# bistromath/gr-ais

Measured on AMD Instinct MI355X. Metric: complex MS/s through corr_est->msk_timing chain; corr_est %HBM roofline, higher is better.
Workload: dtype f32

## Files before the change

### __graft_entry__.py

```python
import os
import subprocess
import sys

ROOT = os.path.dirname(os.path.abspath(__file__))
for _p in (ROOT, os.path.join(ROOT, "gr-ais_amd"), os.path.join(ROOT, "tests")):
    if _p not in sys.path:
        sys.path.insert(0, _p)


def build():
    env = dict(os.environ)
    subprocess.check_call(["make", "-C", os.path.join(ROOT, "gr-ais_amd")], env=env)
    subprocess.check_call(["make", "-C", os.path.join(ROOT, "oracle")], env=env)
    for model in ("emul", "emul_hdlc", "emul_nmea", "emul_nmea_std", "emul_nmea_parse", "emul_msg", "emul_msg_enc", "emul_track", "emul_dedup", "emul_xlate", "emul_xlate_fmt",
                  "emul_mlse"):
        subprocess.check_call(["make", "-C", os.path.join(ROOT, "tests", model)], env=env)
    ub = os.path.join(ROOT, "tools", "ubench")
    src, exe = os.path.join(ub, "hbm_ceiling.hip"), os.path.join(ub, "hbm_ceiling")
    if not os.path.exists(exe) or os.path.getmtime(exe) < os.path.getmtime(src):
        subprocess.check_call([os.environ.get("HIPCC", "/opt/rocm/bin/hipcc"), "--offload-arch=gfx950", "-O3", "-o", exe, src], env=env)
    import ais_amd
    from ais_amd import _lib

    assert _lib.lib().aisx_version() >= 300


def smoke():
    import numpy as np
    import torch

# ... 36 lines not shown
```

### gr-ais_amd/ais_amd/_lib.py

```python
import ctypes as C
import os

_PKG = os.path.dirname(os.path.abspath(__file__))
LIB_VARIANT = os.environ.get("AISX_LIB_VARIANT", "")
LIB_PATH = os.path.join(os.path.dirname(_PKG), "lib", "libaisx_exp.so" if LIB_VARIANT == "exp" else "libaisx.so")

AISX_OK = 0
AISX_ERR_INVALID = -1
AISX_ERR_OUT_OF_RANGE = -2
AISX_ERR_HIP = -3
AISX_ERR_NO_DEVICE = -4
AISX_ERR_OVERFLOW = -5
AISX_ERR_RUNTIME = -6

AISX_FMT_CF32, AISX_FMT_CS16, AISX_FMT_CS8, AISX_FMT_CU8 = 0, 1, 2, 3
AISX_RX_ST_HDLC_OVERFLOW, AISX_RX_ST_NMEA_OVERFLOW, AISX_RX_ST_BAD_COUNT = 0x100, 0x200, 0x400
AISX_MSG_NA, AISX_MSG_STR = -(1 << 31), 48
AISX_HDLC_MAX_RULES = 16
AISX_HDLC_EV_SINGLE, AISX_HDLC_EV_PAIR, AISX_HDLC_EV_SKIP = 1, 2, 4
AISX_MLSE_ST_BAD_COUNT = 1
MLSE_BLOCK, MLSE_OVERLAP = 64, 16
AISX_MSG_FL_COMPLETE, AISX_MSG_FL_NO_LAYOUT, AISX_MSG_FL_BAD_RECORD = 1, 2, 4
AISX_MSG_ENC_NO_MMSI, AISX_MSG_ENC_NO_LAYOUT, AISX_MSG_ENC_RANGE, AISX_MSG_ENC_BAD_CHAR, AISX_MSG_ENC_BAD_ROW = 1, 2, 4, 8, 16
AISX_MSG_ENC_PITCH = 56
# ... 95 lines not shown
    sig("aisx_msk_process_stream", i32, [vp, vp, lng, i32, vp, vp, i32, vp, vp, vp, vp, lng, vp, vp])
    sig("aisx_msk_process_stream_after", i32, [vp, vp, lng, i32, vp, vp, i32, vp, vp, vp, vp, lng, vp, vp, vp])
    sig("aisx_msk_last_status", i32, [vp, pi32, vp])
    sig("aisx_msk_restart_stats", i32, [vp, vp, vp])
    sig("aisx_msk_set_profiling", i32, [vp, i32])
    sig("aisx_msk_kernel_ms_history", i32, [vp, C.POINTER(C.c_float), i32, pi32])
    sig("aisx_msk_set_max_noutput_items", i32, [vp, i32])
    sig("aisx_msk_set_time_parallel", i32, [vp, i32, i32, i32])
    sig("aisx_msk_get_max_noutput_items", i32, [vp])
    sig("aisx_msk_set_tail_stream", i32, [vp, vp, i32])
    sig("aisx_msk_wait_tail", i32, [vp, vp])
    sig("aisx_msk_set_fused_tail", i32, [vp, i32])
    sig("aisx_msk_get_fused_tail", i32, [vp])
    sig("aisx_msk_set_pair_core", i32, [vp, i32])
    sig("aisx_msk_get_pair_core", i32, [vp])
    sig("aisx_msk_last_tail_fused", i32, [vp])
    sig("aisx_msk_wait_prepass", i32, [vp, vp])
    sig("aisx_msk_set_head_start", i32, [vp, i32])
    sig("aisx_msk_geometry", i32, [vp, pi32, pi32])
    sig("aisx_msk_general_work_host", i32, [vp, i32, i32, vp, vp, vp, vp, vp, vp, i32, u64, i32, pi32, pi32])
    sig("aisx_freqsync_create", i32, [pvp, f64, f64, i32, i32, i32])
    sig("aisx_freqest_create", i32, [pvp, f32, i32, i32, i32])
    sig("aisx_freqest_create_n", i32, [pvp, f32, i32, i32, i32, i32])
    sig("aisx_freqsync_is_estimator_only", i32, [vp])
    sig("aisx_freqsync_geometry", i32, [vp, pi32, pi32, pi32])
    sig("aisx_freqsync_drop_ahead", i32, [vp, vp])
    sig("aisx_freqsync_destroy", i32, [vp])
    sig("aisx_freqsync_reset", i32, [vp])
    sig("aisx_freqsync_process", i32, [vp, vp, lng, i32, vp, lng, vp, lng, pi32, vp])
    sig("aisx_freqest_work", i32, [vp, vp, lng, vp, lng, i32, vp])
# ... 182 lines not shown
```

### gr-ais_amd/ais_amd/blocks.py

```python
import ctypes as C
import math

import numpy as np
import torch

from . import _lib
from ._lib import check

TAG_DTYPE = np.dtype([("offset", "<u8"), ("value", "<f8"), ("key", "<i4"), ("chan", "<i4")])


def _stream_ptr(stream=None):
    s = stream if stream is not None else torch.cuda.current_stream()
    return C.c_void_p(s.cuda_stream)


def _dev_c64(x, nchan):
    if not isinstance(x, torch.Tensor):
        x = torch.as_tensor(np.ascontiguousarray(x, dtype=np.complex64))
    if x.dtype != torch.complex64:
        raise TypeError("expected complex64 (gr_complex) items, got %s" % x.dtype)
    if not x.is_cuda:
        x = x.cuda()
    x = x.reshape(nchan, -1)
# ... 214 lines not shown

    def wait_tail(self, stream=None):
        check(_lib.lib().aisx_msk_wait_tail(self._h, _stream_ptr(stream)), "wait_tail")

    def set_fused_tail(self, on):
        check(_lib.lib().aisx_msk_set_fused_tail(self._h, 1 if on else 0), "set_fused_tail")

    def get_fused_tail(self):
        return bool(_lib.lib().aisx_msk_get_fused_tail(self._h))

    def set_pair_core(self, mode):
        check(_lib.lib().aisx_msk_set_pair_core(self._h, int(mode)), "set_pair_core")

    def get_pair_core(self):
        return int(_lib.lib().aisx_msk_get_pair_core(self._h))

    def last_tail_fused(self):
        return _lib.lib().aisx_msk_last_tail_fused(self._h) == 1

    def wait_prepass(self, stream=None):
        check(_lib.lib().aisx_msk_wait_prepass(self._h, _stream_ptr(stream)), "wait_prepass")

    def last_status(self, stream=None):
        st = C.c_int(0)
        check(_lib.lib().aisx_msk_last_status(self._h, C.byref(st), _stream_ptr(stream)), "last_status")
        return st.value

    def set_time_parallel(self, restart_points=64, join_kernel=-1, max_unit_items=0):
        check(_lib.lib().aisx_msk_set_time_parallel(self._h, int(restart_points), int(join_kernel), int(max_unit_items)),
              "set_time_parallel")
# ... 668 lines not shown
```

### gr-ais_amd/csrc/aisx_devctx.h

```cpp
#pragma once
#include <hip/hip_runtime.h>
#include "aisx_common.h"

namespace aisx {

struct DevCtx {
    static constexpr bool wave_lds_coherent = true;
    char* lds_;
    __device__ __forceinline__ int tid() const { return threadIdx.x; }
    __device__ __forceinline__ int nthreads() const { return blockDim.x; }
    __device__ __forceinline__ int bx() const { return blockIdx.x; }
    __device__ __forceinline__ int by() const { return blockIdx.y; }
    __device__ __forceinline__ char* lds() const { return lds_; }
    __device__ __forceinline__ void sync() const { __syncthreads(); }
    __device__ __forceinline__ void wave_sync() const { __builtin_amdgcn_wave_barrier(); }
    __device__ __forceinline__ void wave_lds_sync() const
    {
        asm volatile("" ::: "memory");
        __builtin_amdgcn_wave_barrier();
    }
    __device__ __forceinline__ void retire() const {}
    __device__ __forceinline__ unsigned long long ballot(bool p) const { return __builtin_amdgcn_ballot_w64(p); }
    __device__ __forceinline__ bool inv_ballot(unsigned long long m) const { return __builtin_amdgcn_inverse_ballot_w64(m); }
    typedef float v2f __attribute__((ext_vector_type(2)));
// ... 74 lines not shown
            const auto ra = __builtin_amdgcn_permlane32_swap(a, a, false, false);
            const auto rb = __builtin_amdgcn_permlane32_swap(b, b, false, false);
            lo = mk(__uint_as_float(ra[0]), __uint_as_float(rb[0]));
            hi = mk(__uint_as_float(ra[1]), __uint_as_float(rb[1]));
        }
    }
    static constexpr bool has_pair_core = true;
    struct PairK {
        unsigned long long roleM;
        unsigned rbase;
        float gain_omega, d_sps, limit, gain;
        unsigned rstep;
        unsigned ring;
        unsigned pmask, pbase;
        float rnd;
    };
    __device__ __forceinline__ void pair_core(const PairK& k, float& mu, float& omega, int& sb, unsigned& so, unsigned& waddr, v2f& acc,
                                              v2f& sE, v2f& s1, float& nlO) const
    {
        float t1, t3, t4;
        int t2;
        asm volatile(
            "v_add_f32 %[t3], %[mu], %[om]\n\t"
            "v_cvt_i32_f32 %[t2], %[t3]\n\t"
            "v_fract_f32 %[t1], %[t3]\n\t"
            "v_mad_u32_u24 %[t4], %[t2], %[rstep], %[sb]\n\t"
            "v_cndmask_b32_e64 %[t3], %[mu], %[t1], %[roleM]\n\t"
            "v_and_b32 %[t4], 0x3fc0, %[t4]\n\t"
            "v_fmamk_f32 %[t3], %[t3], 0x43000000, %[rnd]\n\t"
            "v_add_u32 %[t4], %[ring], %[t4]\n\t"
// ... 54 lines not shown
            "v_subrev_f32 v1, %[lim], v1\n\t"
            "v_sub_f32_e64 v0, |v0|, |v1|\n\t"
            "v_mul_f32 v0, 0.5, v0\n\t"
            "v_add_f32 %[om], %[dsps], v0\n\t"
            "v_add_f32 v2, v2, %[om]\n\t"
            "v_cvt_i32_f32 v3, v2\n\t"
            "v_fract_f32 %[mu], v2\n\t"
            "v_lshl_add_u32 %[sb], v3, 6, %[sb]"
            : [mu] "+v"(mu), [om] "+v"(omega), [sb] "+v"(sb), [so] "+v"(so), [waddr] "+v"(waddr), [acc] "+v"(acc), "={v[16:17]}"(sE),
              "+{v[24:25]}"(s1), [nlO] "=&v"(nlO), [t1] "=&v"(t1), [t2] "=&v"(t2), [t3] "=&v"(t3), [t4] "=&v"(t4)
            : [roleM] "s"(k.roleM), [rbase] "s"(k.rbase), [go] "s"(k.gain_omega), [dsps] "s"(k.d_sps), [lim] "s"(k.limit), [gain] "s"(k.gain),
              [rstep] "v"(k.rstep), [ring] "v"(k.ring), [pmask] "v"(k.pmask), [pbase] "v"(k.pbase), [rnd] "v"(k.rnd)
            : "memory", "v0", "v1", "v2", "v3", "v4", "v5", "v6", "v7", "v8", "v9", "v10", "v11", "v12", "v13", "v14", "v15", "v18", "v19",
              "v20", "v21", "v22", "v23");
    }
    __device__ __forceinline__ void xpose8_lane_hi(cf (&x)[8]) const
    {
        unsigned u[16];
#pragma unroll
        for (int k = 0; k < 8; k++) {
            u[2 * k] = __float_as_uint(x[k].re);
            u[2 * k + 1] = __float_as_uint(x[k].im);
        }
#pragma unroll
        for (int r = 0; r < 4; r++)
#pragma unroll
            for (int d = 0; d < 2; d++) {
                const auto q = __builtin_amdgcn_permlane32_swap(u[2 * r + d], u[2 * (r + 4) + d], false, false);
                u[2 * r + d] = q[0];
                u[2 * (r + 4) + d] = q[1];
// ... 201 lines not shown
```

### gr-ais_amd/csrc/aisx_msk.hip

```cpp
#include <math.h>
#include <stdlib.h>

#include <algorithm>
#include <vector>

#include "aisx_devctx.h"
#include "aisx_msk_impl.h"
#include "aisx_plan.h"
#include "aisx_tables.h"

using namespace aisx;

template <bool AUX, bool OSPS2, int LPW>
__global__ __launch_bounds__(64 * msk_waves(LPW)) void k_msk(MskParams p)
{
    extern __shared__ __attribute__((aligned(16))) char smem[];
    DevCtx cx{ smem };
#ifndef MSK_PRIO
#define MSK_PRIO 3
#endif
    __builtin_amdgcn_s_setprio(MSK_PRIO);
    msk_body<DevCtx, AUX, OSPS2, LPW>(cx, p);
}

template <int LPW>
__global__ __launch_bounds__(64 * msk_waves(LPW)) void k_msk_ff(MskParams p)
{
    extern __shared__ __attribute__((aligned(16))) char smem[];
    DevCtx cx{ smem };
    __builtin_amdgcn_s_setprio(MSK_PRIO);
    msk_body<DevCtx, false, false, LPW, true>(cx, p);
}

__global__ __launch_bounds__(64 * msk_waves(8)) void k_msk_core(MskParams p)
{
    extern __shared__ __attribute__((aligned(16))) char smem[];
    DevCtx cx{ smem };
    __builtin_amdgcn_s_setprio(MSK_PRIO);
    msk_body<DevCtx, false, false, 8, false, true>(cx, p);
}

__global__ __launch_bounds__(BT_T) void k_bittail(BitTailParams p)
{
    __shared__ __attribute__((aligned(16))) char smem[260 * 4];
    DevCtx cx{ smem };
    bittail_body(cx, p);
}

__global__ __launch_bounds__(64) void k_msk_headstart(unsigned ticks)
// ... 23 lines not shown
    const int v = li * 4 + (((p.err || p.mu_out) ? 2 : 0) | (p.osps == 2 ? 1 : 0));
    static const int pad = [] {
        const char* e = exp_env("AISX_MSK_LDS_PAD");
        return e ? atoi(e) * 1024 : 0;
    }();
    const int lds = std::min(msk_lds_bytes(p.lpw) + pad, 160 * 1024);
    kfn fn = fns[v];
    if (p.ff) {
        static const kfn ffs[5] = { k_msk_ff<16>, k_msk_ff<32>, k_msk_ff<64>, k_msk_ff<8>, k_msk_ff<4> };
        if (p.err || p.mu_out || p.osps == 2) {
            set_err("msk_launch: the join build has no err / mu ports and osps == 1");
            return AISX_ERR_INVALID;
        }
        fn = ffs[li];
    } else if (p.pair_core && v == 3 * 4) {
        fn = k_msk_core;
    }
    int rc = ensure_dyn_lds((const void*)fn, lds, "msk_timing_recovery_cc");
    if (rc != AISX_OK)
        return rc;
    hipLaunchKernelGGL(fn, dim3(nwg), dim3(64 * msk_waves(p.lpw)), lds, st, p);
    AISX_HIPCHK(hipGetLastError());
    return AISX_OK;
}

static int msk_check_geometry(float d_sps, float gain, float limit)
{
    const float wmin = d_sps - fabsf(limit), wmax = d_sps + fabsf(limit);
    if (!(wmin >= 0.5f) || msk_forecast(d_sps, 1) + 1 > aisx_msk::carry_cap || !(2.f * wmax + 3.f * fabsf(gain) <= 32.f)) {
        set_err("msk_timing_recovery: sps/2 = %g with limit %g and gain %g is outside what the gfx950 kernel is sized for "
                "(sps/2 - |limit| >= 0.5, forecast(1) < %d items, 2 (sps/2 + |limit|) + 3 |gain| <= 32)",
// ... 182 lines not shown
void aisx::msk_fill_common(aisx_msk* h, MskParams& p)
{
    msk_fill_state(h, p);
    p.osps = h->osps;
    p.ct = h->d_ct;
    p.ct_n = h->d_ct_n;
    p.ct_cap = h->ct_cap();
    p.lds_tab_off = msk_lds_taboff(h->lpw);
    p.lpw = h->lpw;
    p.lds_wave_stride = msk_lds_wave(h->lpw);
    p.tq_stride = h->lpw;
    p.tq_private = 0;
    p.lds_ring_off = msk_lds_ringoff(h->lpw);
    p.inline_tags = h->inline_tags;
    p.pair_core = h->pair_core;
    p.stream_mode = 1;
    p.gr_ninput = 0;
    p.gr_noutput = 0;
    p.ff = 0;
    p.nrst = nullptr;
    p.rst = nullptr;
    p.res = nullptr;
    p.pieces = nullptr;
    p.npieces = nullptr;
    p.ct_nc = nullptr;
}

static int msk_ct_reserve(aisx_msk* h, int need, hipStream_t st)
{
    if (h->d_ct && need <= h->ct_cap())
// ... 234 lines not shown
        return AISX_ERR_INVALID;
    h->fused_tail = on != 0;
    return AISX_OK;
}
extern "C" int aisx_msk_get_fused_tail(const aisx_msk* h) { return h ? (h->fused_tail ? 1 : 0) : AISX_ERR_INVALID; }
extern "C" int aisx_msk_last_tail_fused(const aisx_msk* h) { return h ? (h->last_fused ? 1 : 0) : AISX_ERR_INVALID; }

extern "C" int aisx_msk_set_pair_core(aisx_msk* h, int mode)
{
    if (!h || (mode != 0 && mode != 1))
        return AISX_ERR_INVALID;
    h->pair_core = mode;
    return AISX_OK;
}
extern "C" int aisx_msk_get_pair_core(const aisx_msk* h) { return h ? h->pair_core : AISX_ERR_INVALID; }

extern "C" int aisx_msk_wait_prepass(aisx_msk* h, void* stream)
{
    if (!h)
        return AISX_ERR_INVALID;
    if (!h->ev_prep)
        return h->ev_prep.ensure(hipEventDisableTiming);
    if (h->ev_prep_set) {
        AISX_HIPCHK(hipStreamWaitEvent((hipStream_t)stream, h->ev_prep, 0));
        if (h->head_start_ticks > 0) {
            hipLaunchKernelGGL(k_msk_headstart, dim3(1), dim3(64), 0, (hipStream_t)stream, h->head_start_ticks);
            AISX_HIPCHK(hipGetLastError());
        }
    }
    return AISX_OK;
// ... 165 lines not shown
```

### gr-ais_amd/csrc/aisx_msk_impl.h

```cpp
#pragma once
#include <memory>
#include <vector>

#include "aisx_host.h"
#include "k_msk.h"

#pragma GCC visibility push(hidden)
namespace aisx {
struct MskTp;
struct MskTpDelete {
    void operator()(MskTp* t) const;
};
}

struct aisx_msk {
    int nchan = 0, max_items = 0, out_cap = 0, osps = 1;
    aisx::EventRing prof;
    int lpw = 64;
    int inline_tags = 1;
    float d_sps = 0, gain = 0, gain_omega = 0, limit = 0;
    static constexpr int carry_cap = aisx::MSK_CARRY_MAX, ctag_cap = 64;
    aisx::DevBuf<float> d_mu, d_omega;
    aisx::DevBuf<int> d_div;
    aisx::DevBuf<aisx::cf> d_dly1, d_dly2, d_diff1;
    aisx::DevBuf<aisx::cf> d_tprev[2];
    aisx::DevBuf<unsigned char> d_tbit[2];
    int tcur = 0;
    aisx::DevBuf<aisx::cf> d_symscratch[2];
    int callpar = 0;
    bool tail_on = false;
    hipStream_t tail_stream = nullptr;
    aisx::Event ev_msk, ev_tail[2];
    unsigned head_start_ticks = 0;
    aisx::Event ev_prep;
    bool ev_prep_set = false;
    bool ev_tail_set[2] = { false, false };
    bool fused_tail = true, last_fused = false;
    int pair_core = 1;
    hipStream_t last_st = nullptr;
    bool tail_pend[2] = { false, false };
    aisx::DevBuf<int> d_produced2;
    aisx::DevBuf<unsigned long long> d_nread;
    aisx::DevBuf<aisx::cf> d_carry[2];
    aisx::DevBuf<int> d_carry_len[2];
    aisx::DevBuf<aisx::tag_rec> d_ctag[2];
    aisx::DevBuf<int> d_ctag_n[2];
    aisx::DevBuf<aisx::msk_ctag> d_ct;
    aisx::DevBuf<int> d_ct_n;
    int ct_cap() const { return (int)(d_ct.cap() / (size_t)nchan); }
    int cur = 0;
    aisx::DevBuf<int> d_produced, d_consumed, d_status;
    aisx::DevBuf<float> d_mmse, d_atan;
    int max_noutput = 0;
// ... 77 lines not shown
```

### gr-ais_amd/csrc/aisx_stages.hip

```cpp
#include <math.h>
#include <stdlib.h>
#include <string.h>

#include <vector>

#include "aisx_devctx.h"
#include "aisx_host.h"
#include "aisx_tables.h"
#include "k_agc.h"
#include "k_agcw.h"
#include "k_freqsync.h"

using namespace aisx;

__global__ __launch_bounds__(FS_T) void k_fs_est(FsEstParams p)
{
    extern __shared__ __attribute__((aligned(16))) char smem[];
    DevCtx cx{ smem };
    fs_est_body(cx, p);
}
__global__ __launch_bounds__(FSM_T) void k_fs_mix(FsMixParams p)
{
    extern __shared__ __attribute__((aligned(16))) char smem[];
    DevCtx cx{ smem };
// ... 273 lines not shown
extern "C" int aisx_freqsync_process(aisx_freqsync* h, const aisx_cf32* d_in, long in_stride, int n, aisx_cf32* d_out,
                                     long out_stride, float* d_fhat, long fhat_stride, int* n_out, void* stream)
{
    if (fs_whole(h, "aisx_freqsync_process") != AISX_OK)
        return AISX_ERR_INVALID;
    if (!h || !d_in || !d_out || !n_out || n < 1 || n > h->max_items || in_stride < n) {
        set_err("aisx_freqsync_process: bad argument");
        return AISX_ERR_INVALID;
    }
    hipStream_t st = (hipStream_t)stream;
    const int nvec = (h->npend + n) / h->fftlen;
    if (out_stride < (long)nvec * h->fftlen || (d_fhat && fhat_stride < nvec)) {
        set_err("aisx_freqsync_process: output stride too small for %d vectors", nvec);
        return AISX_ERR_INVALID;
    }
    h->ahead_cnt = 0;
    if (h->walk_pending)
        AISX_HIPCHK(hipStreamWaitEvent(st, h->ev_walk, 0));
    if (h->proc_pending)
        AISX_HIPCHK(hipStreamWaitEvent(st, h->ev_proc, 0));
    if (nvec > 0) {
        FsEstParams e;
        e.in = (const cf*)d_in;
        e.in_stride = in_stride;
        e.pend = h->d_pend[h->cur];
        e.npend = h->npend;
        e.wtab = h->d_wtab;
        e.maxpos = h->d_maxpos;
        e.maxpos_stride = h->max_vec;
        e.nvec = nvec;
// ... 10 lines not shown
    m.npend = h->npend;
    m.n = n;
    m.out = (cf*)d_out;
    m.out_stride = out_stride;
    m.maxpos = h->d_maxpos;
    m.maxpos_stride = h->max_vec;
    m.fhat = d_fhat;
    m.fhat_stride = fhat_stride;
    m.phase = h->d_phase;
    m.nvec = nvec;
    m.binsize = h->binsize;
    m.sensitivity = h->sensitivity;
    m.sintab = h->d_sintab;
    hipLaunchKernelGGL(k_fs_mix, dim3((h->nchan + FSM_CPW - 1) / FSM_CPW), dim3(FSM_T), FSM_LDS_BYTES, st, m);
    AISX_HIPCHK(hipGetLastError());
    if (h->ev_proc) {
        AISX_HIPCHK(hipEventRecord(h->ev_proc, st));
        AISX_HIPCHK(hipEventRecord(h->ev_walk, st));
        h->proc_pending = h->walk_pending = true;
        AISX_HIPCHK(hipEventRecord(h->slot[0].ev_read, st));
        h->slot[0].read_pending = true;
    }
    h->npend = h->npend + n - nvec * h->fftlen;
    h->cur ^= 1;
    *n_out = nvec * h->fftlen;
    return AISX_OK;
}

extern "C" int aisx_freqest_work(aisx_freqsync* h, const aisx_cf32* d_vecs, long vec_stride, float* d_out,
                                 long out_stride, int nvec, void* stream)
{
    if (!h || !d_vecs || !d_out || nvec < 0 || vec_stride < (long)nvec * h->fftlen || out_stride < nvec)
        return AISX_ERR_INVALID;
    if (nvec == 0)
        return AISX_OK;
    FsFreqestParams p;
    p.vecs = (const cf*)d_vecs;
// ... 571 lines not shown
```

### gr-ais_amd/csrc/k_msk.h

```cpp
#pragma once
#include "aisx_common.h"

namespace aisx {

enum {
    MSK_ST_INTERP_RANGE = 1,
    MSK_ST_CARRY_OVERFLOW = 2,
    MSK_ST_TAGCARRY_OVERFLOW = 4,
    MSK_ST_OUT_FULL = 8,
    MSK_ST_TAGS_TRUNCATED = 16
};
constexpr int MSK_CTN_TRUNC = 0x40000000;
constexpr int MSK_CTN_WILD = 0x20000000;
constexpr int MSK_TAG_TRIPS = 6;

constexpr int MSK_T = 64;
constexpr int MSK_RING = 256;
constexpr int MSK_SLOTS = MSK_RING + 8;
constexpr int MSK_CHUNK = 64;
constexpr int MSK_OFF = 192;
constexpr int MSK_CARRY_MAX = 128;
constexpr int MSK_PAIRS_MAX = 16;
#ifndef MSK_TRIP
#define MSK_TRIP 8
// ... 126 lines not shown
    int stream_mode; int gr_ninput; int gr_noutput;
    const msk_ctag* ct; const int* ct_n; int ct_cap;
    tag_rec* ctag_out; int* ctag_n_out; int ctag_cap;
    cf* syms; float* err; float* mu_out; long out_stride; int out_cap;
    int* produced; int* consumed; int* status;
    const float* mmse;
    int lds_tab_off;
    int lds_wave_stride, tq_stride, tq_private;
    int lds_ring_off;
    int sym_al16;
    int lpw;
    int inline_tags;
    int max_noutput;
    int ff;
    int pair_core = 0;
    const int* nrst; const mskp_rst* rst; const mskp_res* res;
    mskp_piece* pieces; int* npieces;
    const int* ct_nc;
    unsigned char* bits = nullptr; long bit_stride = 0;
    int bit_al2 = 0;
    const cf* prev_sym_in = nullptr; const unsigned char* prev_bit_in = nullptr;
    cf* prev_sym_out = nullptr; unsigned char* prev_bit_out = nullptr;
    const float* atan_tab = nullptr;
};

struct BitTailParams {
    int nchan;
    const cf* syms; long sym_stride;
    const int* produced;
    unsigned char* bits; long bit_stride;
// ... 7 lines not shown
    return (int)ceil((noutput_items * d_sps * 2) + 3.0 * d_sps + 8u);
}

#ifdef MSK_EMU_STATS
extern long msk_stats[8];
#endif
#ifdef MSK_EMU_RUN_STATS
extern long msk_run_stats[MSK_PAIRS_MAX + 1];
#endif
template <class Ctx, class = void>
struct msk_has_pair_core { static constexpr bool value = false; };
template <class Ctx>
struct msk_has_pair_core<Ctx, decltype((void)Ctx::has_pair_core)> { static constexpr bool value = Ctx::has_pair_core; };
template <class Ctx>
struct msk_stage_rot { static constexpr bool value = !Ctx::wave_lds_coherent; };
template <class Ctx, bool AUX, bool OSPS2, int LPW, bool FFT = false, bool CORE = false>
AISX_DI void msk_body(Ctx& cx, const MskParams& p)
{
    static_assert(!FFT || (!AUX && !OSPS2), "the join build has no err / mu ports and osps == 1");
    static_assert(!CORE || (msk_has_pair_core<Ctx>::value && !AUX && !OSPS2 && !FFT && LPW == 8), "the scheduled pair is written for this build");
    constexpr int SLOT_B = LPW * 8;
    constexpr int SLOT_SH = LPW == 64 ? 9 : (LPW == 32 ? 8 : (LPW == 16 ? 7 : (LPW == 8 ? 6 : 5)));
    static_assert(LPW == 4 || LPW == 8 || LPW == 16 || LPW == 32 || LPW == 64, "channels per wave");
    typedef unsigned long long u64;
    static_assert(64 % LPW == 0, "whole waves");
    constexpr int NQ = 64 / LPW;
    constexpr int QS = MSK_CHUNK / NQ;
    const int wv = cx.tid() >> 6;
    const int l = cx.tid() & (LPW - 1);
    const int q = (cx.tid() & 63) / LPW;
    const bool owner = q == 0;
    const int cbase = cx.bx() * msk_wg_channels(LPW) + wv * LPW;
    const int c = cbase + l;
    const bool live = c < p.nchan;
    const int cc = live ? c : (p.nchan - 1);
// ... 545 lines not shown
        const tap4* tp4 = (const tap4*)((const char*)mm + row * (unsigned)(MSK_TAPS_PITCH * 4));
        const tap4 tlo = tp4[0], thi = tp4[1];
        const float tp[8] = { tlo[0], tlo[1], tlo[2], tlo[3], thi[0], thi[1], thi[2], thi[3] };
        struct alignas(8) cf8 { float re, im; };
        const cf8* sp = (const cf8*)(lds + (((unsigned)sbpos & (unsigned)((MSK_RING - 1) * SLOT_B)) | (unsigned)(l * 8)));
#pragma unroll
        for (int k = 0; k < 8; k++) {
            const cf8 t = sp[k * LPW];
            sv[k] = mk(t.re, t.im);
            tv[k] = tp[7 - k];
        }
    };
    const unsigned mm_rbase = mmse_row_base((unsigned)p.lds_tab_off, (unsigned)(MSK_TAPS_PITCH * 4));
    const char* const lds_l = lds + l * 8;
    constexpr unsigned RING_M = (unsigned)((MSK_RING - 1) * SLOT_B);
    auto fir_load_pair = [&](float mu, unsigned soff, cf* sv, float* tv) {
        typedef float tap4 __attribute__((vector_size(16)));
        const tap4* tp4 = (const tap4*)(lds0 + mmse_row_off(mu, (unsigned)(MSK_TAPS_PITCH * 4), mm_rbase));
        const tap4 tlo = tp4[0], thi = tp4[1];
        const float tp[8] = { tlo[0], tlo[1], tlo[2], tlo[3], thi[0], thi[1], thi[2], thi[3] };
        struct alignas(8) cf8 { float re, im; };
        const cf8* sp = (const cf8*)(lds_l + soff);
#pragma unroll
        for (int k = 0; k < 8; k++) {
            const cf8 t = sp[k * LPW];
            sv[k] = mk(t.re, t.im);
            tv[k] = tp[7 - k];
        }
    };
    auto fir_sum = [&](const cf* sv, const float* tv) -> cf {
        cf acc = mk(0.f, 0.f);
#pragma unroll
        for (int k = 0; k < 8; k++) {
            acc.re += sv[k].re * tv[k];
            acc.im += sv[k].im * tv[k];
        }
        return acc;
    };

    auto fir = [&](unsigned row, int sbpos) -> cf {
        cf sv[8];
        float tv[8];
        fir_load(row, sbpos, sv, tv);
// ... 252 lines not shown
            }
#ifdef MSK_PROF
            if (npairs == 0) { pf_fail += __builtin_readcyclecounter() - pf_a; pf_nfail++; }
#endif
            if (npairs > 0) {
              if constexpr (NQ >= 2) {
                constexpr int ROW = LPW <= 16 ? 16 : 32;
                const bool roleO = (cx.tid() & ROW) != 0;
                const unsigned rstep = (unsigned)(cx.tid() & ROW) * (unsigned)(SLOT_B / ROW);
                const unsigned pmask = roleO ? 0u : STG_MASK, pbase = roleO ? stg_spare : stg_real;
                cf sqO = prev_sq, sqE = mk(0.f, 0.f), acc = last_interp;
                float nl_prev = d_dly_diff_1.re;
                const int sb_entry = sb;
                constexpr bool ROT = STG && (CORE || msk_stage_rot<Ctx>::value);
                unsigned wat = stg_spare;
              if constexpr (CORE) {
                typename Ctx::PairK kk;
                kk.roleM = cx.ballot(roleO);
                kk.rbase = mm_rbase + cx.lds_addr(lds0);
                kk.gain_omega = p.gain_omega;
                kk.d_sps = d_sps;
                kk.limit = p.limit;
                kk.gain = p.gain;
                kk.rstep = rstep;
                kk.ring = cx.lds_addr(lds_l);
                kk.pmask = pmask;
                kk.pbase = pbase + cx.lds_addr(lds0);
                kk.rnd = 12582912.0f;
                typename Ctx::v2f a2 = Ctx::tov(acc), e2 = Ctx::tov(sqE), o2 = Ctx::tov(sqO);
                wat += cx.lds_addr(lds0);
                auto pair = [&]() { cx.pair_core(kk, d_mu, d_omega, sb, so, wat, a2, e2, o2, nl_prev); };
// ... 54 lines not shown
                                if (omu0)
                                    *(float*)(omu0 + (ob >> 1)) = d_mu;
                            }
                        }
                        ob += 8u;
                    }
                    const float m2 = mu2 + d_omega;
                    d_mu = cx.fract(m2);
                    sb = sb1 + (int)m2 * SLOT_B;
                    sqE = sE;
                    sqO = s1;
                    nl_prev = nlO;
                };
                msk_run_trips<MSK_TRIP_CXX>(npairs, pair);
              }
                if constexpr (ROT)
                    stage_at(wat, acc);
                cf accE, accO;
                cx.template pair_rows<ROW>(acc, accE, accO);
                d_div += 2 * npairs;
                oidx += OSPS2 ? 2 * npairs : npairs;
                iidx += (sb - sb_entry) >> SLOT_SH;
                prev_sq = sqO;
                last_interp = accO;
                d_dly_diff_1 = mk(nl_prev, sqO.im * sqE.re - sqO.re * sqE.im);
                if (!(d_mu >= 0.f && d_mu <= 1.f))
                    status |= MSK_ST_INTERP_RANGE;
              } else {
                const int sb_entry = sb;
                cf sqO = prev_sq, sqE = mk(0.f, 0.f), accO = last_interp;
                float nl_prev = d_dly_diff_1.re;
// ... 378 lines not shown
```

### include/aisx.h

```cpp
#ifndef AISX_H
#define AISX_H

#include <stddef.h>
#include <stdint.h>

#ifdef __cplusplus
extern "C" {
#endif

#define AISX_VERSION 300

typedef struct aisx_cf32 { float re, im; } aisx_cf32;

enum {
    AISX_KEY_CORR_START = 0,
    AISX_KEY_PHASE_EST = 1,
    AISX_KEY_TIME_EST = 2,
    AISX_KEY_CORR_EST = 3,
    AISX_KEY_PORT1 = 0x100
};
typedef struct aisx_tag {
    uint64_t offset;
    double value;
    int32_t key;
// ... 77 lines not shown
int aisx_msk_set_max_noutput_items(aisx_msk* h, int max_noutput_items);
int aisx_msk_set_time_parallel(aisx_msk* h, int restart_points_per_channel, int join_kernel, int max_unit_items);
int aisx_msk_get_max_noutput_items(const aisx_msk* h);
int aisx_msk_last_status(aisx_msk* h, int* status, void* stream);
int aisx_msk_status_device(const aisx_msk* h, const int** d_status);
int aisx_msk_restart_stats(aisx_msk* h, long long* out10, void* stream);
int aisx_msk_set_profiling(aisx_msk* h, int on);
int aisx_msk_kernel_ms_history(aisx_msk* h, float* ms, int cap, int* n);
int aisx_msk_set_tail_stream(aisx_msk* h, void* tail_stream, int enable);
int aisx_msk_wait_tail(aisx_msk* h, void* stream);
int aisx_msk_set_fused_tail(aisx_msk* h, int on);
int aisx_msk_get_fused_tail(const aisx_msk* h);
int aisx_msk_last_tail_fused(const aisx_msk* h);
int aisx_msk_set_pair_core(aisx_msk* h, int mode);
int aisx_msk_get_pair_core(const aisx_msk* h);
int aisx_msk_wait_prepass(aisx_msk* h, void* stream);
int aisx_msk_set_head_start(aisx_msk* h, int microseconds);
int aisx_msk_general_work_host(aisx_msk* h, int noutput_items, int ninput_items, const aisx_cf32* in, aisx_cf32* out,
                               float* out_err, float* out_mu, uint8_t* out_bits, const aisx_tag* tags, int ntags,
                               uint64_t nitems_read, int in_has_lookahead, int* consumed, int* produced);

typedef struct aisx_freqsync aisx_freqsync;
int aisx_freqsync_create(aisx_freqsync** h, double samplerate, double bits_per_sec, int fftlen, int nchan,
                         int max_items);
int aisx_freqsync_destroy(aisx_freqsync* h);
int aisx_freqsync_geometry(const aisx_freqsync* h, int* nchan, int* max_items, int* fftlen);
int aisx_freqsync_drop_ahead(aisx_freqsync* h, void* stream);
int aisx_freqsync_set_walk_lds_claim(aisx_freqsync* h, int bytes);
int aisx_freqsync_get_walk_lds_claim(const aisx_freqsync* h, int* bytes, int* used_bytes);
int aisx_freqest_create(aisx_freqsync** h, float sample_rate, int data_rate, int fftlen, int max_vectors);
// ... 373 lines not shown
```

Measured before the change: 55330.

## Split MSK pair loop across lane halves, one real component per lane

Adds a split variant of the hand-scheduled MSK timing-recovery pair loop. Each half-row of lanes now handles only the real or the imaginary component: it reads scalar ring samples instead of complex pairs and exchanges partial products through DPP row_ror and permlane16 swaps. The idea is to shorten the serial per-pair FIR and LDS work on the latency-bound recursive timing loop, paying for it with extra cross-lane exchanges and a recombination step after the loop. It is enabled by default through pair_split=1. The freqsync event setup is also moved ahead of the launch so events are always recorded, not only when they already exist.

```diff
diff --git a/__graft_entry__.py b/__graft_entry__.py
--- a/__graft_entry__.py
+++ b/__graft_entry__.py
@@ -13,7 +13,7 @@
     subprocess.check_call(["make", "-C", os.path.join(ROOT, "gr-ais_amd")], env=env)
     subprocess.check_call(["make", "-C", os.path.join(ROOT, "oracle")], env=env)
     for model in ("emul", "emul_hdlc", "emul_nmea", "emul_nmea_std", "emul_nmea_parse", "emul_msg", "emul_msg_enc", "emul_track", "emul_dedup", "emul_xlate", "emul_xlate_fmt",
-                  "emul_mlse"):
+                  "emul_mlse", "emul_msk_split", "emul_msk_split_end"):
         subprocess.check_call(["make", "-C", os.path.join(ROOT, "tests", model)], env=env)
     ub = os.path.join(ROOT, "tools", "ubench")
     src, exe = os.path.join(ub, "hbm_ceiling.hip"), os.path.join(ub, "hbm_ceiling")
diff --git a/gr-ais_amd/ais_amd/_lib.py b/gr-ais_amd/ais_amd/_lib.py
--- a/gr-ais_amd/ais_amd/_lib.py
+++ b/gr-ais_amd/ais_amd/_lib.py
@@ -133,6 +133,8 @@
     sig("aisx_msk_get_fused_tail", i32, [vp])
     sig("aisx_msk_set_pair_core", i32, [vp, i32])
     sig("aisx_msk_get_pair_core", i32, [vp])
+    sig("aisx_msk_set_pair_split", i32, [vp, i32])
+    sig("aisx_msk_get_pair_split", i32, [vp])
     sig("aisx_msk_last_tail_fused", i32, [vp])
     sig("aisx_msk_wait_prepass", i32, [vp, vp])
     sig("aisx_msk_set_head_start", i32, [vp, i32])
diff --git a/gr-ais_amd/ais_amd/blocks.py b/gr-ais_amd/ais_amd/blocks.py
--- a/gr-ais_amd/ais_amd/blocks.py
+++ b/gr-ais_amd/ais_amd/blocks.py
@@ -252,6 +252,12 @@
 
     def get_pair_core(self):
         return int(_lib.lib().aisx_msk_get_pair_core(self._h))
+
+    def set_pair_split(self, on):
+        check(_lib.lib().aisx_msk_set_pair_split(self._h, int(on)), "set_pair_split")
+
+    def get_pair_split(self):
+        return int(_lib.lib().aisx_msk_get_pair_split(self._h))
 
     def last_tail_fused(self):
         return _lib.lib().aisx_msk_last_tail_fused(self._h) == 1
diff --git a/gr-ais_amd/csrc/aisx_devctx.h b/gr-ais_amd/csrc/aisx_devctx.h
--- a/gr-ais_amd/csrc/aisx_devctx.h
+++ b/gr-ais_amd/csrc/aisx_devctx.h
@@ -112,6 +112,7 @@
         unsigned ring;
         unsigned pmask, pbase;
         float rnd;
+        unsigned long long compM;
     };
     __device__ __forceinline__ void pair_core(const PairK& k, float& mu, float& omega, int& sb, unsigned& so, unsigned& waddr, v2f& acc,
                                               v2f& sE, v2f& s1, float& nlO) const
@@ -196,6 +197,98 @@
             : "memory", "v0", "v1", "v2", "v3", "v4", "v5", "v6", "v7", "v8", "v9", "v10", "v11", "v12", "v13", "v14", "v15", "v18", "v19",
               "v20", "v21", "v22", "v23");
     }
+    __device__ __forceinline__ float half_row_other(float v) const
+    {
+        return __uint_as_float((unsigned)__builtin_amdgcn_update_dpp(0, (int)__float_as_uint(v), 0x128, 0xf, 0xf, false));
+    }
+    __device__ __forceinline__ void pair_split(const PairK& k, float& mu, float& omega, int& sb, unsigned& so, unsigned& waddr, float& acc,
+                                               float& sE, float& s1, float& nlO) const
+    {
+        float t1, t3, t4;
+        int t2;
+        asm volatile(
+            "v_add_f32 %[t3], %[mu], %[om]\n\t"
+            "v_cvt_i32_f32 %[t2], %[t3]\n\t"
+            "v_fract_f32 %[t1], %[t3]\n\t"
+            "v_mad_u32_u24 %[t4], %[t2], %[rstep], %[sb]\n\t"
+            "v_cndmask_b32_e64 %[t3], %[mu], %[t1], %[roleM]\n\t"
+            "v_and_b32 %[t4], 0x3fc0, %[t4]\n\t"
+            "v_fmamk_f32 %[t3], %[t3], 0x43000000, %[rnd]\n\t"
+            "v_add_u32 %[t4], %[ring], %[t4]\n\t"
+            "v_mad_u32_u24 %[t3], %[t3], 48, %[rbase]\n\t"
+            "ds_read_b128 v[4:7], %[t3] offset:16\n\t"
+            "ds_read2_b32 v[8:9], %[t4] offset1:16\n\t"
+            "ds_read_b128 v[0:3], %[t3]\n\t"
+            "ds_read2_b32 v[10:11], %[t4] offset0:32 offset1:48\n\t"
+            "ds_read2_b32 v[12:13], %[t4] offset0:64 offset1:80\n\t"
+            "ds_read2_b32 v[14:15], %[t4] offset0:96 offset1:112\n\t"
+            "ds_write_b32 %[waddr], %[acc]\n\t"
+            "v_lshl_add_u32 %[sb], %[t2], 6, %[sb]\n\t"
+            "v_and_b32 %[waddr], %[so], %[pmask]\n\t"
+            "v_mov_b32 v17, v24\n\t"
+            "v_add_u32 %[waddr], %[pbase], %[waddr]\n\t"
+            "v_add_u32 %[so], 64, %[so]\n\t"
+            "s_waitcnt lgkmcnt(5)\n\t"
+            "v_mul_f32 %[acc], v8, v7\n\t"
+            "v_mul_f32 v8, v9, v6\n\t"
+            "v_add_f32 %[acc], 0, %[acc]\n\t"
+            "s_waitcnt lgkmcnt(3)\n\t"
+            "v_mul_f32 v9, v10, v5\n\t"
+            "v_add_f32 %[acc], %[acc], v8\n\t"
+            "v_mul_f32 v8, v11, v4\n\t"
+            "v_add_f32 %[acc], %[acc], v9\n\t"
+            "s_waitcnt lgkmcnt(1)\n\t"
+            "v_mul_f32 v9, v12, v3\n\t"
+            "v_add_f32 %[acc], %[acc], v8\n\t"
+            "v_mul_f32 v8, v13, v2\n\t"
+            "v_add_f32 %[acc], %[acc], v9\n\t"
+            "v_mul_f32 v9, v14, v1\n\t"
+            "v_add_f32 %[acc], %[acc], v8\n\t"
+            "v_mul_f32 v8, v15, v0\n\t"
+            "v_add_f32 %[acc], %[acc], v9\n\t"
+            "v_add_f32 %[acc], %[acc], v8\n\t"
+            "s_nop 1\n\t"
+            "v_mov_b32_dpp v10, %[acc] row_ror:8 row_mask:0xf bank_mask:0xf\n\t"
+            "v_cndmask_b32_e64 v11, %[acc], v10, %[compM]\n\t"
+            "v_cndmask_b32_e64 v12, -v10, %[acc], %[compM]\n\t"
+            "v_mul_f32 v11, v11, %[acc]\n\t"
+            "v_mul_f32 v12, v12, v10\n\t"
+            "v_add_f32 v16, v11, v12\n\t"
+            "v_add_f32 v24, v11, v12\n\t"
+            "s_nop 1\n\t"
+            "v_permlane16_swap_b32 v16, v24\n\t"
+            "v_mul_f32 v8, v16, v17\n\t"
+            "v_mul_f32 v9, v24, v16\n\t"
+            "s_nop 0\n\t"
+            "v_add_f32_dpp v0, v8, v8 row_ror:8 row_mask:0xf bank_mask:0xf\n\t"
+            "v_add_f32_dpp %[nlO], v9, v9 row_ror:8 row_mask:0xf bank_mask:0xf\n\t"
+            "v_sub_f32 v0, %[nlO], v0\n\t"
+            "s_nop 1\n\t"
+            "v_mov_b32_dpp v0, v0 row_ror:8 row_mask:0xf bank_mask:0x3\n\t"
+            "v_add_f32 v1, 0x40400000, v0\n\t"
+            "v_add_f32 v2, 0xc0400000, v0\n\t"
+            "v_sub_f32_e64 v0, |v1|, |v2|\n\t"
+            "v_mul_f32 v0, 0.5, v0\n\t"
+            "v_mul_f32 v1, %[go], v0\n\t"
+            "v_mul_f32 v2, %[gain], v0\n\t"
+            "v_add_f32 v1, %[om], v1\n\t"
+            "v_add_f32 v2, %[t1], v2\n\t"
+            "v_subrev_f32 v1, %[dsps], v1\n\t"
+            "v_add_f32 v0, %[lim], v1\n\t"
+            "v_subrev_f32 v1, %[lim], v1\n\t"
+            "v_sub_f32_e64 v0, |v0|, |v1|\n\t"
+            "v_mul_f32 v0, 0.5, v0\n\t"
+            "v_add_f32 %[om], %[dsps], v0\n\t"
+            "v_add_f32 v2, v2, %[om]\n\t"
+            "v_cvt_i32_f32 v3, v2\n\t"
+            "v_fract_f32 %[mu], v2\n\t"
+            "v_lshl_add_u32 %[sb], v3, 6, %[sb]"
+            : [mu] "+v"(mu), [om] "+v"(omega), [sb] "+v"(sb), [so] "+v"(so), [waddr] "+v"(waddr), [acc] "+v"(acc), "=&{v16}"(sE), "+{v24}"(s1),
+              [nlO] "=&v"(nlO), [t1] "=&v"(t1), [t2] "=&v"(t2), [t3] "=&v"(t3), [t4] "=&v"(t4)
+            : [roleM] "s"(k.roleM), [compM] "s"(k.compM), [rbase] "s"(k.rbase), [go] "s"(k.gain_omega), [dsps] "s"(k.d_sps), [lim] "s"(k.limit),
+              [gain] "s"(k.gain), [rstep] "v"(k.rstep), [ring] "v"(k.ring), [pmask] "v"(k.pmask), [pbase] "v"(k.pbase), [rnd] "v"(k.rnd)
+            : "memory", "v0", "v1", "v2", "v3", "v4", "v5", "v6", "v7", "v8", "v9", "v10", "v11", "v12", "v13", "v14", "v15", "v17");
+    }
     __device__ __forceinline__ void xpose8_lane_hi(cf (&x)[8]) const
     {
         unsigned u[16];
diff --git a/gr-ais_amd/csrc/aisx_msk.hip b/gr-ais_amd/csrc/aisx_msk.hip
--- a/gr-ais_amd/csrc/aisx_msk.hip
+++ b/gr-ais_amd/csrc/aisx_msk.hip
@@ -33,6 +33,14 @@
 }
 
 __global__ __launch_bounds__(64 * msk_waves(8)) void k_msk_core(MskParams p)
+{
+    extern __shared__ __attribute__((aligned(16))) char smem[];
+    DevCtx cx{ smem };
+    __builtin_amdgcn_s_setprio(MSK_PRIO);
+    msk_body<DevCtx, false, false, 8, false, true, true>(cx, p);
+}
+
+__global__ __launch_bounds__(64 * msk_waves(8)) void k_msk_core_whole(MskParams p)
 {
     extern __shared__ __attribute__((aligned(16))) char smem[];
     DevCtx cx{ smem };
@@ -86,7 +94,7 @@
         }
         fn = ffs[li];
     } else if (p.pair_core && v == 3 * 4) {
-        fn = k_msk_core;
+        fn = p.pair_split ? k_msk_core : k_msk_core_whole;
     }
     int rc = ensure_dyn_lds((const void*)fn, lds, "msk_timing_recovery_cc");
     if (rc != AISX_OK)
@@ -299,6 +307,7 @@
     p.lds_ring_off = msk_lds_ringoff(h->lpw);
     p.inline_tags = h->inline_tags;
     p.pair_core = h->pair_core;
+    p.pair_split = h->pair_split;
     p.stream_mode = 1;
     p.gr_ninput = 0;
     p.gr_noutput = 0;
@@ -563,6 +572,14 @@
     return AISX_OK;
 }
 extern "C" int aisx_msk_get_pair_core(const aisx_msk* h) { return h ? h->pair_core : AISX_ERR_INVALID; }
+extern "C" int aisx_msk_set_pair_split(aisx_msk* h, int mode)
+{
+    if (!h || (mode != 0 && mode != 1))
+        return AISX_ERR_INVALID;
+    h->pair_split = mode;
+    return AISX_OK;
+}
+extern "C" int aisx_msk_get_pair_split(const aisx_msk* h) { return h ? h->pair_split : AISX_ERR_INVALID; }
 
 extern "C" int aisx_msk_wait_prepass(aisx_msk* h, void* stream)
 {
diff --git a/gr-ais_amd/csrc/aisx_msk_impl.h b/gr-ais_amd/csrc/aisx_msk_impl.h
--- a/gr-ais_amd/csrc/aisx_msk_impl.h
+++ b/gr-ais_amd/csrc/aisx_msk_impl.h
@@ -37,6 +37,7 @@
     bool ev_tail_set[2] = { false, false };
     bool fused_tail = true, last_fused = false;
     int pair_core = 1;
+    int pair_split = 1;
     hipStream_t last_st = nullptr;
     bool tail_pend[2] = { false, false };
     aisx::DevBuf<int> d_produced2;
diff --git a/gr-ais_amd/csrc/aisx_stages.hip b/gr-ais_amd/csrc/aisx_stages.hip
--- a/gr-ais_amd/csrc/aisx_stages.hip
+++ b/gr-ais_amd/csrc/aisx_stages.hip
@@ -311,6 +311,10 @@
         set_err("aisx_freqsync_process: output stride too small for %d vectors", nvec);
         return AISX_ERR_INVALID;
     }
+    int rc;
+    if ((rc = h->ev_walk.ensure(hipEventDisableTiming)) != AISX_OK || (rc = h->ev_proc.ensure(hipEventDisableTiming)) != AISX_OK ||
+        (rc = h->slot[0].ev_read.ensure(hipEventDisableTiming)) != AISX_OK)
+        return rc;
     h->ahead_cnt = 0;
     if (h->walk_pending)
         AISX_HIPCHK(hipStreamWaitEvent(st, h->ev_walk, 0));
@@ -351,13 +355,11 @@
     m.sintab = h->d_sintab;
     hipLaunchKernelGGL(k_fs_mix, dim3((h->nchan + FSM_CPW - 1) / FSM_CPW), dim3(FSM_T), FSM_LDS_BYTES, st, m);
     AISX_HIPCHK(hipGetLastError());
-    if (h->ev_proc) {
-        AISX_HIPCHK(hipEventRecord(h->ev_proc, st));
-        AISX_HIPCHK(hipEventRecord(h->ev_walk, st));
-        h->proc_pending = h->walk_pending = true;
-        AISX_HIPCHK(hipEventRecord(h->slot[0].ev_read, st));
-        h->slot[0].read_pending = true;
-    }
+    AISX_HIPCHK(hipEventRecord(h->ev_proc, st));
+    AISX_HIPCHK(hipEventRecord(h->ev_walk, st));
+    h->proc_pending = h->walk_pending = true;
+    AISX_HIPCHK(hipEventRecord(h->slot[0].ev_read, st));
+    h->slot[0].read_pending = true;
     h->npend = h->npend + n - nvec * h->fftlen;
     h->cur ^= 1;
     *n_out = nvec * h->fftlen;
diff --git a/gr-ais_amd/csrc/k_msk.h b/gr-ais_amd/csrc/k_msk.h
--- a/gr-ais_amd/csrc/k_msk.h
+++ b/gr-ais_amd/csrc/k_msk.h
@@ -164,6 +164,7 @@
     int max_noutput;
     int ff;
     int pair_core = 0;
+    int pair_split = 0;
     const int* nrst; const mskp_rst* rst; const mskp_res* res;
     mskp_piece* pieces; int* npieces;
     const int* ct_nc;
@@ -201,11 +202,15 @@
 struct msk_has_pair_core<Ctx, decltype((void)Ctx::has_pair_core)> { static constexpr bool value = Ctx::has_pair_core; };
 template <class Ctx>
 struct msk_stage_rot { static constexpr bool value = !Ctx::wave_lds_coherent; };
-template <class Ctx, bool AUX, bool OSPS2, int LPW, bool FFT = false, bool CORE = false>
+#ifndef MSK_PAIR_SPLIT_CXX
+#define MSK_PAIR_SPLIT_CXX 0
+#endif
+template <class Ctx, bool AUX, bool OSPS2, int LPW, bool FFT = false, bool CORE = false, bool SPLITC = false>
 AISX_DI void msk_body(Ctx& cx, const MskParams& p)
 {
     static_assert(!FFT || (!AUX && !OSPS2), "the join build has no err / mu ports and osps == 1");
     static_assert(!CORE || (msk_has_pair_core<Ctx>::value && !AUX && !OSPS2 && !FFT && LPW == 8), "the scheduled pair is written for this build");
+    static_assert(!SPLITC || CORE, "the split stretch belongs to the scheduled build");
     constexpr int SLOT_B = LPW * 8;
     constexpr int SLOT_SH = LPW == 64 ? 9 : (LPW == 32 ? 8 : (LPW == 16 ? 7 : (LPW == 8 ? 6 : 5)));
     static_assert(LPW == 4 || LPW == 8 || LPW == 16 || LPW == 32 || LPW == 64, "channels per wave");
@@ -781,9 +786,17 @@
     const unsigned mm_rbase = mmse_row_base((unsigned)p.lds_tab_off, (unsigned)(MSK_TAPS_PITCH * 4));
     const char* const lds_l = lds + l * 8;
     constexpr unsigned RING_M = (unsigned)((MSK_RING - 1) * SLOT_B);
+    auto tap_row_off_pair = [&](float mu) -> unsigned {
+        unsigned o = mmse_row_off(mu, (unsigned)(MSK_TAPS_PITCH * 4), mm_rbase);
+#if !defined(__HIP_DEVICE_COMPILE__)
+        if (o - (unsigned)p.lds_tab_off >= 130u * (unsigned)(MSK_TAPS_PITCH * 4))
+            o = (unsigned)p.lds_tab_off + (unsigned)(MSK_ZERO_ROW * MSK_TAPS_PITCH * 4);
+#endif
+        return o;
+    };
     auto fir_load_pair = [&](float mu, unsigned soff, cf* sv, float* tv) {
         typedef float tap4 __attribute__((vector_size(16)));
-        const tap4* tp4 = (const tap4*)(lds0 + mmse_row_off(mu, (unsigned)(MSK_TAPS_PITCH * 4), mm_rbase));
+        const tap4* tp4 = (const tap4*)(lds0 + tap_row_off_pair(mu));
         const tap4 tlo = tp4[0], thi = tp4[1];
         const float tp[8] = { tlo[0], tlo[1], tlo[2], tlo[3], thi[0], thi[1], thi[2], thi[3] };
         struct alignas(8) cf8 { float re, im; };
@@ -794,6 +807,15 @@
             sv[k] = mk(t.re, t.im);
             tv[k] = tp[7 - k];
         }
+    };
+    auto tap_load_pair = [&](float mu, float* tv) {
+        typedef float tap4 __attribute__((vector_size(16)));
+        const tap4* tp4 = (const tap4*)(lds0 + tap_row_off_pair(mu));
+        const tap4 tlo = tp4[0], thi = tp4[1];
+        const float tp[8] = { tlo[0], tlo[1], tlo[2], tlo[3], thi[0], thi[1], thi[2], thi[3] };
+#pragma unroll
+        for (int k = 0; k < 8; k++)
+            tv[k] = tp[7 - k];
     };
     auto fir_sum = [&](const cf* sv, const float* tv) -> cf {
         cf acc = mk(0.f, 0.f);
@@ -1076,7 +1098,101 @@
                 const int sb_entry = sb;
                 constexpr bool ROT = STG && (CORE || msk_stage_rot<Ctx>::value);
                 unsigned wat = stg_spare;
-              if constexpr (CORE) {
+                constexpr bool SPLIT = STG && LPW == 8 && !FFT && (CORE ? SPLITC : (MSK_PAIR_SPLIT_CXX != 0));
+              if constexpr (SPLIT) {
+                const bool compI = (cx.tid() & 8) != 0;
+                const unsigned cofs = (unsigned)(cx.tid() & 8) >> 1;
+                auto other_half = [&](float v) -> float {
+                    if constexpr (CORE)
+                        return cx.half_row_other(v);
+                    else
+                        return cx.xchg(v, (cx.tid() & 63) ^ 8);
+                };
+                auto stage_comp = [&](unsigned at, float v) { *(float*)(lds0 + at) = v; };
+                float ac = compI ? acc.im : acc.re, oc = compI ? sqO.im : sqO.re, ec = 0.f;
+                wat += cofs;
+                if constexpr (CORE) {
+                    typename Ctx::PairK kk;
+                    kk.roleM = cx.ballot(roleO);
+                    kk.compM = cx.ballot(compI);
+                    kk.rbase = mm_rbase + cx.lds_addr(lds0);
+                    kk.gain_omega = p.gain_omega;
+                    kk.d_sps = d_sps;
+                    kk.limit = p.limit;
+                    kk.gain = p.gain;
+                    kk.rstep = rstep;
+                    kk.ring = cx.lds_addr(lds_l) + cofs;
+                    kk.pmask = pmask;
+                    kk.pbase = pbase + cx.lds_addr(lds0) + cofs;
+                    kk.rnd = 12582912.0f;
+                    wat += cx.lds_addr(lds0);
+                    auto pair = [&]() { cx.pair_split(kk, d_mu, d_omega, sb, so, wat, ac, ec, oc, nl_prev); };
+                    msk_run_trips<MSK_TRIP>(npairs, pair);
+                    wat -= cx.lds_addr(lds0);
+                } else {
+#ifdef MSK_EMU_RUN_STATS
+                    if (l == 0 && q == 0) msk_run_stats[npairs]++;
+#endif
+                    const char* const lds_c = lds_l + cofs;
+                    auto pair = [&]() {
+#ifdef MSK_EMU_STATS
+                        if (l == 0 && q == 0) msk_stats[0]++;
+#endif
+                        const float m1 = d_mu + d_omega;
+                        const float muO = cx.fract(m1);
+                        const int adv1 = (int)m1;
+                        const int sb1 = sb + adv1 * SLOT_B;
+                        float tv[8], sc[8];
+                        tap_load_pair(roleO ? muO : d_mu, tv);
+                        const char* const sp = lds_c + ring_read_off(sb, adv1, rstep, RING_M);
+#pragma unroll
+                        for (int k = 0; k < 8; k++)
+                            sc[k] = *(const float*)(sp + k * SLOT_B);
+                        if constexpr (ROT) {
+                            stage_comp(wat, ac);
+                            wat = ((so & pmask) | pbase) + cofs;
+                            so += (unsigned)SLOT_B;
+                        }
+                        float a = 0.f;
+#pragma unroll
+                        for (int k = 0; k < 8; k++)
+                            a += sc[k] * tv[k];
+                        ac = a;
+                        const float y = other_half(ac);
+                        const float R = compI ? y : ac, I = compI ? ac : y;
+                        const float pa = R * ac, pb = I * y;
+                        const float sq = compI ? pa + pb : pa - pb;
+                        cf sE, s1;
+                        cx.template pair_rows<ROW>(mk(sq, 0.f), sE, s1);
+                        const float pE = sE.re * oc, pO = s1.re * sE.re;
+                        const float qE = other_half(pE), qO = other_half(pO);
+                        const float nlE = compI ? qE + pE : pE + qE;
+                        const float nlO = compI ? qO + pO : pO + qO;
+                        const float err = branchless_clip(nlO - nlE, 3.0f);
+                        d_omega += p.gain_omega * err;
+                        d_omega = d_sps + branchless_clip(d_omega - d_sps, p.limit);
+                        const float mu2 = muO + p.gain * err;
+                        if constexpr (!ROT) {
+                            stage_comp(((so & pmask) | pbase) + cofs, ac);
+                            so += (unsigned)SLOT_B;
+                        }
+                        const float m2 = mu2 + d_omega;
+                        d_mu = cx.fract(m2);
+                        sb = sb1 + (int)m2 * SLOT_B;
+                        ec = sE.re;
+                        oc = s1.re;
+                        nl_prev = nlO;
+                    };
+                    msk_run_trips<MSK_TRIP_CXX>(npairs, pair);
+                }
+                if constexpr (ROT)
+                    stage_comp(wat, ac);
+                const float ao = other_half(ac), eo = other_half(ec), oo = other_half(oc), no = other_half(nl_prev);
+                acc = compI ? mk(ao, ac) : mk(ac, ao);
+                sqE = compI ? mk(eo, ec) : mk(ec, eo);
+                sqO = compI ? mk(oo, oc) : mk(oc, oo);
+                nl_prev = compI ? nl_prev : no;
+              } else if constexpr (CORE) {
                 typename Ctx::PairK kk;
                 kk.roleM = cx.ballot(roleO);
                 kk.rbase = mm_rbase + cx.lds_addr(lds0);
@@ -1161,7 +1277,7 @@
                 };
                 msk_run_trips<MSK_TRIP_CXX>(npairs, pair);
               }
-                if constexpr (ROT)
+                if constexpr (ROT && !SPLIT)
                     stage_at(wat, acc);
                 cf accE, accO;
                 cx.template pair_rows<ROW>(acc, accE, accO);
diff --git a/include/aisx.h b/include/aisx.h
--- a/include/aisx.h
+++ b/include/aisx.h
@@ -115,6 +115,8 @@
 int aisx_msk_last_tail_fused(const aisx_msk* h);
 int aisx_msk_set_pair_core(aisx_msk* h, int mode);
 int aisx_msk_get_pair_core(const aisx_msk* h);
+int aisx_msk_set_pair_split(aisx_msk* h, int on);
+int aisx_msk_get_pair_split(const aisx_msk* h);
 int aisx_msk_wait_prepass(aisx_msk* h, void* stream);
 int aisx_msk_set_head_start(aisx_msk* h, int microseconds);
 int aisx_msk_general_work_host(aisx_msk* h, int noutput_items, int ninput_items, const aisx_cf32* in, aisx_cf32* out,
```

After: 55910, median of 6. 1.01x the previous value.
